# YPares/gaast

Measured on AMD Instinct MI355X. Metric: full-MV geometric products/sec (dim n); achieved HBM GB/s vs roofline, higher is better.
Workload: dtype f32; 1 GPU; R^12 full MV x MV geometric product, f32 (BASELINE configs[2]); dim=12, batch_per_gpu=65536, global_batch=65536

## Files before the change

gaast_amd/csrc/device/kernels_dense.hip.hpp:

```cpp
#pragma once
#include "kernels_common.hip.hpp"
#include "mfma32p_b_planes.hip.hpp"


namespace gaast {

template <typename T>
struct DenseArgs {
    const T* left;
    const T* right;
    T* out;
    int64_t left_stride, right_stride, out_stride;
    const uint32_t* left_map;
    const uint32_t* right_map;
    int left_count, right_count;
    int left_full, right_full;
    int left_contig, right_contig;
    const int32_t* out_map;
    int canon_left, canon_right;
    int n;
    uint32_t neg_hi, zero_hi;
    uint32_t neg_lo;
    int beta;
    const T* left_scale;
// ... 402 lines not shown
            auto one_step = [&](auto odd_tag, int a_hi) {
                constexpr bool ODD = decltype(odd_tag)::value;
                uint32_t sp = uint32_t(a_hi) >> 1;
                sp ^= sp >> 1;
                sp ^= sp >> 2;
                sp ^= sp >> 4;
                sp ^= sp >> 8;
                const uint32_t M = sp ^ (uint32_t(a_hi) & p.neg_hi);
                const uint32_t u = (__builtin_popcount(uint32_t(a_hi) & sp) ^
                                    __builtin_popcount(uint32_t(a_hi) & p.neg_hi)) & 1u;
                const uint32_t sbit = (u ^ uint32_t(__builtin_popcount(uint32_t(c_hi) & M))) & 1u;
                T sgn = sbit ? T(-1) : T(1);
                if (DEGENERATE) {
                    if (uint32_t(a_hi) & ~uint32_t(c_hi) & p.zero_hi) sgn = zero;
                }
                acc.template step<ODD, NEGLO>(As, Bs, a_hi, a_hi ^ c_hi, sgn);
            };
            const int half = LPI >> 1;
            for (int i = 0; i < half; ++i) one_step(std::false_type{}, (i << 1) | (__builtin_popcount(uint32_t(i)) & 1));
            for (int i = 0; i < half; ++i) one_step(std::true_type{}, (i << 1) | ((__builtin_popcount(uint32_t(i)) & 1) ^ 1));

            T* orow = p.out + (item0 + it) * p.out_stride;
#pragma unroll
            for (int i = 0; i < 16; ++i) store_result<T>(orow, om[i], acc.get(i), p.beta, out_scale, (c_hi << 4) + i);
        }
        __syncthreads();
    }
}


__device__ __forceinline__ constexpr int lo5_reorder_parity(int a, int b) {
    int par = 0;
    for (int p = 1; p < 5; ++p)
        if ((a >> p) & 1)
            for (int q = 0; q < p; ++q) par ^= (b >> q) & 1;
    return par;
}

__device__ __forceinline__ int mfma_b_pos(int m) {
    const int x = m >> 5, k = m & 31;
    const int lq = ((k & 1) << 2) | (k >> 3);
    return (x << 5) | (((lq ^ (x >> 1)) & 7) << 2) | ((k >> 1) & 3);
}

template <bool DEGENERATE, int THREADS, bool SCALED = false, bool CHAINED = false>
__global__ __launch_bounds__(THREADS) void k_gp_mfma32(DenseArgs<float> p) {
    const float* const left_scale = SCALED ? p.left_scale : nullptr;
    const float* const right_scale = SCALED ? p.right_scale : nullptr;
    const float* const out_scale = SCALED ? p.out_scale : nullptr;
    extern __shared__ __attribute__((aligned(16))) unsigned char smem_raw[];
    float* smem = reinterpret_cast<float*>(smem_raw);
    const int n = p.n;
    const int N = 1 << n;
    const int hbits = n - 5;
    const int H = 1 << hbits;
    const int WPI = H >> 5;
    const int IPB = (THREADS >> 6) / WPI;
    const int item_stride = 2 * N;
    const int tid = threadIdx.x;
    const int64_t item0 = int64_t(blockIdx.x) * IPB;
    const int nitems = int(p.batch - item0 < IPB ? p.batch - item0 : IPB);

    if (!p.left_full || !p.right_full) {
        for (int i = tid; i < nitems * item_stride; i += THREADS) smem[i] = 0.f;
        __syncthreads();
    }
    {
        if constexpr (CHAINED)
            stage_from_list<float, THREADS>(p, item0, nitems, smem, item_stride, smem + p.pre_scratch, tid);
        else
            stage_operands<float, THREADS>(p.left + item0 * p.left_stride, p.left_stride, p.left_map, p.left_count, p.left_contig,
                                       p.canon_left, smem, item_stride, nitems, tid, left_scale);
        stage_operands<float, THREADS>(p.right + item0 * p.right_stride, p.right_stride, p.right_map, p.right_count,
                                       p.right_contig, p.canon_right, smem + N, item_stride, nitems, tid, right_scale);
    }
    __syncthreads();

    const int wave = tid >> 6, lane = tid & 63;
    const int it = wave / WPI, tile = wave - it * WPI;
    if (it < nitems) {
        const float* As = smem + it * item_stride;
        const float* Bs = As + N;
        const int i = lane & 31, h = lane >> 5;
        const int c_hi = (tile << 5) | i;

        uint32_t amask[16];
        uint32_t aoff[16];
#pragma unroll
        for (int s2 = 0; s2 < 16; ++s2) {
            const int k = 2 * s2 + h;
            const int a_lo = i ^ k;
            int par = __builtin_popcount(uint32_t(a_lo & k) & p.neg_lo) & 1;
            for (int pp = 1; pp < 5; ++pp)
                if ((a_lo >> pp) & 1) par ^= __builtin_popcount(k & ((1 << pp) - 1)) & 1;
            amask[s2] = uint32_t(par) << 31;
            aoff[s2] = uint32_t(a_lo) << 2;
        }

        float16v acc;
#pragma unroll
        for (int r = 0; r < 16; ++r) acc[r] = 0.f;

        const unsigned char* As_b = reinterpret_cast<const unsigned char*>(As);
        const unsigned char* Bs_b = reinterpret_cast<const unsigned char*>(Bs);
        uint32_t bq[4];
#pragma unroll
        for (int q = 0; q < 4; ++q) bq[q] = (uint32_t(c_hi) << 7) | (uint32_t((((h << 2) | q) ^ (c_hi >> 1)) & 7) << 4);
        const uint32_t c_hi_u = uint32_t(c_hi) | 0x8000u;
        auto one_step = [&](int a_hi) {
            uint32_t sp = uint32_t(a_hi) >> 1;
            sp ^= sp >> 1;
            sp ^= sp >> 2;
            sp ^= sp >> 4;
            sp ^= sp >> 8;
            const uint32_t M = sp ^ (uint32_t(a_hi) & p.neg_hi);
            const uint32_t u = (__builtin_popcount(uint32_t(a_hi) & sp) ^
                                __builtin_popcount(uint32_t(a_hi) & p.neg_hi)) & 1u;
            const uint32_t bmask = uint32_t(__builtin_popcount(c_hi_u & (M | (u << 15)))) << 31;
            float bscale = 1.f;
            if (DEGENERATE) {
                if (uint32_t(a_hi) & ~uint32_t(c_hi) & p.zero_hi) bscale = 0.f;
            }
            float bv[16];
            const uint32_t sx = (uint32_t(a_hi) << 7) | (uint32_t((a_hi >> 1) & 7) << 4);
#pragma unroll
            for (int q = 0; q < 4; ++q) {
                const float4v v = *reinterpret_cast<const float4v*>(Bs_b + (bq[q] ^ sx));
                bv[4 * q + 0] = v.x; bv[4 * q + 1] = v.y; bv[4 * q + 2] = v.z; bv[4 * q + 3] = v.w;
            }
            const uint32_t abase = uint32_t(a_hi) << 7;
#pragma unroll
            for (int s2 = 0; s2 < 16; ++s2) {
                float a = *reinterpret_cast<const float*>(As_b + abase + aoff[s2]);
                a = __uint_as_float(__float_as_uint(a) ^ amask[s2]);
                float b = __uint_as_float(__float_as_uint(bv[s2]) ^ bmask);
                if (DEGENERATE) b *= bscale;
                acc = __builtin_amdgcn_mfma_f32_32x32x2f32(a, b, acc, 0, 0, 0);
            }
        };
        const int half = H >> 1;
        for (int t2 = 0; t2 < half; ++t2) one_step((t2 << 1) | (__builtin_popcount(uint32_t(t2)) & 1));
#pragma unroll
        for (int s2 = 0; s2 < 16; ++s2)
            amask[s2] ^= uint32_t((__builtin_popcount(uint32_t(s2)) + h) & 1) << 31;
        for (int t2 = 0; t2 < half; ++t2) one_step((t2 << 1) | ((__builtin_popcount(uint32_t(t2)) & 1) ^ 1));

        float* orow = p.out + (item0 + it) * p.out_stride;
        const int32_t* om = p.out_map + (c_hi << 5);
#pragma unroll
        for (int r = 0; r < 16; ++r) {
            const int c_lo = (r & 3) + 8 * (r >> 2) + 4 * h;
            store_result<float>(orow, om[c_lo], acc[r], p.beta, out_scale, (c_hi << 5) + c_lo);
        }
    }
}

template <int THREADS>
__device__ __forceinline__ void lds_barrier() {
    if (THREADS <= 64) {
        __builtin_amdgcn_wave_barrier();
        asm volatile("" ::: "memory");
    } else {
        asm volatile("s_waitcnt lgkmcnt(0)\n\ts_barrier" ::: "memory");
    }
}

typedef __attribute__((address_space(3))) unsigned char lds_u8;
typedef uint32_t uint4v __attribute__((ext_vector_type(4)));

__device__ __forceinline__ uint32_t xor3(uint32_t a, uint32_t b, uint32_t c) {
#if __has_builtin(__builtin_amdgcn_bitop3_b32)
    return __builtin_amdgcn_bitop3_b32(a, b, c, 0x96);
#else
    return a ^ b ^ c;
#endif
}

__device__ __forceinline__ constexpr int mfma16_k(int t) {
    constexpr int order[16] = {0, 3, 5, 6, 9, 10, 12, 15, 1, 2, 4, 7, 8, 11, 13, 14};
    return order[t];
}
static_assert(mfma16_k(1) == int(b_planes::s2_of_word(1)) && mfma16_k(7) == int(b_planes::s2_of_word(7)) && mfma16_k(8) == int(b_planes::s2_of_word(8)) &&
              mfma16_k(14) == int(b_planes::s2_of_word(14)), "the quad-plane B image stores the words in mfma16_k order");

template <bool DEGENERATE, int NDIM, bool SCALED = false, bool CHAINED = false>
__global__ __launch_bounds__(NDIM == 13 ? 512 : 256, NDIM <= 11 ? 2 : 1) void k_gp_mfma32p(DenseArgs<float> p) {
    const float* const left_scale = SCALED ? p.left_scale : nullptr;
    const float* const right_scale = SCALED ? p.right_scale : nullptr;
    const float* const out_scale = SCALED ? p.out_scale : nullptr;
    extern __shared__ __attribute__((aligned(16))) unsigned char smem_raw[];
    float* smem = reinterpret_cast<float*>(smem_raw);
    lds_u8* lds = (lds_u8*)smem_raw;
    constexpr int n = NDIM;
    constexpr int THREADS = NDIM == 13 ? 512 : 256;
    constexpr int N = 1 << n;
    constexpr int H = 1 << (n - 5);
    constexpr int WPI = H >> 5;
    constexpr int IPB = (THREADS >> 6) / WPI;
    constexpr int item_stride = 4 * N;
    constexpr uint32_t NEG = uint32_t(N) << 2;
    constexpr int PR = N / 4;
    constexpr int MPR = PR / THREADS;
    constexpr int ROWS = 2 * IPB;
    static_assert(MPR * ROWS == 8, "eight 16-byte pieces per thread and group");
    const int tid = threadIdx.x;
    const int64_t num_groups = (p.batch + IPB - 1) / IPB;
    const bool fast = !SCALED && !CHAINED && p.left_contig && p.right_contig && p.left_full && p.right_full;

    if (tid < 16) smem[IPB * item_stride + tid] = 0.f;

    uint32_t mw[2][MPR * 4];
    float4 pf[8];
    auto fetch = [&](int64_t g) {
        const int64_t it0 = g * IPB;
        const int cnt = int(p.batch - it0 < IPB ? p.batch - it0 : IPB);
#pragma unroll
        for (int r = 0; r < ROWS; ++r) {
            const int k = r % IPB;
            if (k < cnt) {
                const float* row = r < IPB ? p.left + (it0 + k) * p.left_stride : p.right + (it0 + k) * p.right_stride;
#pragma unroll
                for (int m = 0; m < MPR; ++m) pf[r * MPR + m] = reinterpret_cast<const float4*>(row)[tid + m * THREADS];
            }
        }
    };
    if (fast) {
#pragma unroll
        for (int m = 0; m < MPR; ++m) {
            const uint4 ml = reinterpret_cast<const uint4*>(p.left_map)[tid + m * THREADS];
            const uint4 mr = reinterpret_cast<const uint4*>(p.right_map)[tid + m * THREADS];
            mw[0][4 * m + 0] = ml.x; mw[0][4 * m + 1] = ml.y; mw[0][4 * m + 2] = ml.z; mw[0][4 * m + 3] = ml.w;
            mw[1][4 * m + 0] = mr.x; mw[1][4 * m + 1] = mr.y; mw[1][4 * m + 2] = mr.z; mw[1][4 * m + 3] = mr.w;
        }
        if (int64_t(blockIdx.x) < num_groups) fetch(blockIdx.x);
    }

    const int wave = tid >> 6, lane = tid & 63;
    const int it = wave / WPI, tile = wave - it * WPI;
    const int i = lane & 31, h = lane >> 5;
    const int c_hi = (tile << 5) | i;
    const uint32_t item_base = uint32_t(it) * uint32_t(item_stride) * 4u;

    constexpr bool ABS_A = NDIM <= 11 || (NDIM == 12 && !DEGENERATE);
    const uint32_t lds0 = ABS_A ? uint32_t(size_t(lds)) : 0u;
    uint32_t ak0[16];
#pragma unroll
    for (int t = 0; t < 16; ++t) {
        const int k = 2 * mfma16_k(t) + h;
        const int a_lo = i ^ k;
        int par = __builtin_popcount(uint32_t(a_lo & k) & p.neg_lo) & 1;
        for (int pp = 1; pp < 5; ++pp)
            if ((a_lo >> pp) & 1) par ^= __builtin_popcount(k & ((1 << pp) - 1)) & 1;
        ak0[t] = lds0 + item_base + (uint32_t(a_lo) << 2) + (par ? NEG : 0u);
    }
    const uint32_t b_base = item_base + 2u * NEG;
    constexpr uint32_t zero_block = uint32_t(IPB) * uint32_t(item_stride) * 4u;
    uint32_t bq[4];
#pragma unroll
    for (int q = 0; q < 4; ++q) {
        bq[q] = (uint32_t(c_hi) << 7) | (uint32_t((((h << 2) | q) ^ (c_hi >> 1)) & 7) << 4);
        if ((__builtin_popcount(uint32_t(c_hi)) & 1) && (((q >> 1) ^ h) & 1)) bq[q] ^= NEG;
    }
    const uint32_t c_hi_u = uint32_t(c_hi) | 0x8000u;
    auto sign_terms = [&](int a_hi, uint32_t& M, uint32_t& u) {
        const uint32_t sp = b_planes::suffix_parities(uint32_t(a_hi));
        M = sp ^ (uint32_t(a_hi) & p.neg_hi);
        u = (__builtin_popcount(uint32_t(a_hi) & sp) ^ __builtin_popcount(uint32_t(a_hi) & p.neg_hi)) & 1u;
    };
    auto block_sign = [&](int a_hi) -> uint32_t {
        uint32_t M, u;
        sign_terms(a_hi, M, u);
        return uint32_t(__builtin_popcount(c_hi_u & (M | (u << 15)))) & 1u;
    };
    constexpr int SIGN_WORDS = H <= 64 ? H / 32 : 0;
    constexpr bool XOR_STEP = NDIM == 12 && !DEGENERATE;
    if (XOR_STEP && (lds0 & ((16u << n) - 1u))) __builtin_trap();
    uint32_t dlt[XOR_STEP ? 7 : 1] = {0};
    uint32_t ud[XOR_STEP ? H / 32 : 1] = {0};
    if constexpr (XOR_STEP) {
#pragma unroll
        for (int t = 0; t < 7; ++t) dlt[t] = b_planes::delta(t, uint32_t(c_hi), p.neg_hi);
        static_assert(!XOR_STEP || (NEG == b_planes::kNeg && IPB == 1), "one item per workgroup, the -B image 16 KiB above +B");
#pragma unroll
        for (int w = 0; w < H / 32; ++w) {
            uint32_t bits = 0;
#pragma unroll 1
            for (int b = 0; b < 32; ++b) {
                uint32_t M, u0, u1;
                sign_terms(32 * w + b, M, u0);
                sign_terms(32 * w + b + 1, M, u1);
                bits |= (u0 ^ u1) << b;
            }
            ud[w] = __builtin_amdgcn_readfirstlane(bits);
        }
    }
    uint32_t sgn[SIGN_WORDS > 0 ? SIGN_WORDS : 1] = {0};
#pragma unroll
    for (int w = 0; w < SIGN_WORDS; ++w) {
        uint32_t bits = 0;
#pragma unroll 1
        for (int b = 0; b < 32; ++b) bits |= block_sign(32 * w + b) << b;
        sgn[w] = bits;
    }

    for (int64_t g = blockIdx.x; g < num_groups; g += gridDim.x) {
        const int64_t item0 = g * IPB;
        const int nitems = int(p.batch - item0 < IPB ? p.batch - item0 : IPB);
        if (fast) {
            auto stage_row = [&](int r, bool canon) {
                const int k = r % IPB, side = r / IPB;
                if (k < nitems) {
#pragma unroll
                    for (int m = 0; m < MPR; ++m) {
                        const float4 v = pf[r * MPR + m];
                        const float x[4] = {v.x, v.y, v.z, v.w};
#pragma unroll
                        for (int c = 0; c < 4; ++c) {
                            const uint32_t w = mw[side][4 * m + c];
                            float y = x[c];
                            if (canon) y = 0.f + y;
                            const uint32_t yb = __float_as_uint(y) ^ (w & 0x80000000u);
                            const uint32_t at = uint32_t(k) * uint32_t(item_stride * 4) + (side ? 2u * NEG : 0u) + (((w >> 16) & 0x7fffu) << 2);
                            *(__attribute__((address_space(3))) uint32_t*)(lds + at) = yb;
                            *(__attribute__((address_space(3))) uint32_t*)(lds + at + NEG) = yb ^ 0x80000000u;
                        }
                    }
                }
            };
#pragma unroll
            for (int r = 0; r < ROWS; ++r) {
                if constexpr (XOR_STEP) {
                    if (r / IPB ? p.canon_right : p.canon_left) stage_row(r, true);
                    else stage_row(r, false);
                } else {
                    stage_row(r, r / IPB ? p.canon_right : p.canon_left);
                }
            }
        } else {
            if (!p.left_full || !p.right_full) {
                for (int e = tid; e < nitems * item_stride; e += THREADS) smem[e] = 0.f;
                lds_barrier<THREADS>();
            }
            if constexpr (CHAINED)
                stage_from_list<float, THREADS>(p, item0, nitems, smem, item_stride, smem + p.pre_scratch, tid);
            else
                stage_operands<float, THREADS>(p.left + item0 * p.left_stride, p.left_stride, p.left_map, p.left_count, p.left_contig,
                                           p.canon_left, smem, item_stride, nitems, tid, left_scale);
            stage_operands<float, THREADS>(p.right + item0 * p.right_stride, p.right_stride, p.right_map, p.right_count,
                                           p.right_contig, p.canon_right, smem + 2 * N, item_stride, nitems, tid, right_scale);
            lds_barrier<THREADS>();
            constexpr int quads_per_item = N >> 1;
            for (int e = tid; e < nitems * quads_per_item; e += THREADS) {
                const int sit = e / quads_per_item, j = e - sit * quads_per_item;
                const int src = sit * item_stride + (j << 2) + ((j << 2) < N ? 0 : N);
                const float4v v = *reinterpret_cast<const float4v*>(smem + src);
                *reinterpret_cast<float4v*>(smem + src + N) = -v;
            }
        }
        lds_barrier<THREADS>();
        if (fast && g + gridDim.x < num_groups) fetch(g + gridDim.x);

        if (it < nitems) {
            float16v acc;
#pragma unroll
            for (int r = 0; r < 16; ++r) acc[r] = 0.f;
            uint32_t akc[XOR_STEP ? 1 : 16];
            uint32_t (&ak)[16] = *reinterpret_cast<uint32_t (*)[16]>(XOR_STEP ? ak0 : akc);
            if constexpr (!XOR_STEP) {
#pragma unroll
                for (int t = 0; t < 16; ++t) ak[t] = ak0[t];
            }

            auto step = [&](int a_hi, int j, uint32_t sxs) {
                uint32_t bw[16], aw[16];
#pragma unroll
                for (int q = 0; q < 4; ++q) {
                    uint32_t addr = b_base + (bq[q] ^ sxs);
                    if (DEGENERATE) addr = (uint32_t(a_hi) & ~uint32_t(c_hi) & p.zero_hi) ? zero_block : addr;
                    const uint4v v = *(__attribute__((address_space(3))) const uint4v*)(lds + addr);
                    bw[4 * q + 0] = v.x; bw[4 * q + 1] = v.y; bw[4 * q + 2] = v.z; bw[4 * q + 3] = v.w;
                }
#pragma unroll
                for (int t = 0; t < 16; ++t)
                    aw[t] = ABS_A ? *(__attribute__((address_space(3))) const uint32_t*)size_t(ak[t] + uint32_t(j << 7))
                                  : *(__attribute__((address_space(3))) const uint32_t*)(lds + ak[t] + uint32_t(j << 7));
#pragma unroll
                for (int t = 0; t < 16; ++t)
                    acc = __builtin_amdgcn_mfma_f32_32x32x2f32(__uint_as_float(aw[t]), __uint_as_float(bw[t]), acc, 0, 0, 0);
                asm volatile("" ::: "memory");
            };
            if constexpr (SIGN_WORDS > 0 && NDIM <= 11) {
                uint32_t awin[4];
                uint4v qb[2];
                auto b_quad = [&](int a_hi, int q, uint32_t sxs) -> uint4v {
                    uint32_t addr = b_base + (bq[q] ^ sxs);
                    if (DEGENERATE) addr = (uint32_t(a_hi) & ~uint32_t(c_hi) & p.zero_hi) ? zero_block : addr;
                    return *(__attribute__((address_space(3))) const uint4v*)(lds + addr);
                };
                auto a_word = [&](int t, int j) -> uint32_t {
                    return ABS_A ? *(__attribute__((address_space(3))) const uint32_t*)size_t(ak[t] + uint32_t(j << 7))
                                 : *(__attribute__((address_space(3))) const uint32_t*)(lds + ak[t] + uint32_t(j << 7));
                };
                auto sx_of = [&](int a_hi) -> uint32_t {
                    uint32_t sx = __builtin_amdgcn_readfirstlane((uint32_t(a_hi) << 7) | (uint32_t((a_hi >> 1) & 7) << 4));
                    asm("" : "+s"(sx));
                    return sx;
                };
                uint32_t sxs = ((sgn[0] & 1u) << (n + 2)) | sx_of(0);
                qb[0] = b_quad(0, 0, sxs);
#pragma unroll
                for (int t = 0; t < 3; ++t) awin[t] = a_word(t, 0);
#pragma unroll
                for (int w = 0; w < SIGN_WORDS; ++w) {
                    uint32_t sw = sgn[w];
                    const uint32_t next_word_bit0 = w + 1 < SIGN_WORDS ? (sgn[w + 1 < SIGN_WORDS ? w + 1 : w] & 1u) : 0u;
#pragma unroll 1
                    for (int c = 0; c < 2; ++c) {
                        const int a0 = 32 * w + 16 * c;
#pragma unroll
                        for (int j = 0; j < 16; ++j) {
                            const int a_hi = a0 + j;
                            const uint32_t nbit = j < 15 ? (sw >> (j + 1)) & 1u : (c == 0 ? (sw >> 16) & 1u : next_word_bit0);
                            const uint32_t nsxs = (nbit << (n + 2)) | sx_of(a_hi + 1);
#pragma unroll
                            for (int t = 0; t < 16; ++t) {
                                const int m = 16 * j + t;
                                const int t3 = (t + 3) & 15, j3 = j + ((t + 3) >> 4);
                                awin[(m + 3) & 3] = a_word(t3, j3);
                                if ((t & 3) == 0) {
                                    const int q = t >> 2;
                                    qb[(q + 1) & 1] = q < 3 ? b_quad(a_hi, q + 1, sxs) : b_quad(a_hi + 1, 0, nsxs);
                                }
                                __builtin_amdgcn_sched_barrier(0);
                                const uint4v bqv = qb[(t >> 2) & 1];
                                const uint32_t bwv = (t & 3) == 0 ? bqv.x : (t & 3) == 1 ? bqv.y : (t & 3) == 2 ? bqv.z : bqv.w;
                                acc = __builtin_amdgcn_mfma_f32_32x32x2f32(__uint_as_float(awin[m & 3]), __uint_as_float(bwv), acc, 0, 0, 0);
                                __builtin_amdgcn_sched_barrier(0);
                            }
                            sxs = nsxs;
                        }
                        sw >>= 16;
#pragma unroll
                        for (int t = 0; t < 16; ++t) ak[t] += 16u << 7;
                    }
                }
            } else if constexpr (XOR_STEP) {
                uint32_t xe = lds0 + (b_base | b_planes::xe0(uint32_t(c_hi), uint32_t(h)));
                uint32_t xo = lds0 + (b_base | b_planes::xo0(uint32_t(c_hi), uint32_t(h)));
#pragma unroll 1
                for (int c = 0; c < H / 64; ++c) {
                    const uint32_t udw[2] = {c == 0 ? ud[0] : ud[2], c == 0 ? ud[1] : ud[3]};
#pragma unroll
                    for (int j = 0; j < 64; ++j) {
                        uint32_t bw[16], aw[16];
#pragma unroll
                        for (int q = 0; q < 4; ++q) {
                            const uint4v v = *(__attribute__((address_space(3))) const uint4v*)size_t((q & 2 ? xo : xe) + uint32_t(q & 1) * b_planes::kQuadStride);
                            bw[4 * q + 0] = v.x; bw[4 * q + 1] = v.y; bw[4 * q + 2] = v.z; bw[4 * q + 3] = v.w;
                        }
#pragma unroll
                        for (int t = 0; t < 16; ++t)
                            aw[t] = *(__attribute__((address_space(3))) const uint32_t*)size_t(ak[t] + uint32_t(j << 7));
#pragma unroll
                        for (int t = 0; t < 16; ++t)
                            acc = __builtin_amdgcn_mfma_f32_32x32x2f32(__uint_as_float(aw[t]), __uint_as_float(bw[t]), acc, 0, 0, 0);
                        asm volatile("" ::: "memory");
                        uint32_t su = __builtin_amdgcn_readfirstlane(((udw[j >> 5] >> (j & 31)) & 1u) << (n + 2));
                        asm("" : "+s"(su));
                        const uint32_t d = dlt[j < 63 ? __builtin_ctz(~uint32_t(j)) : 6];
                        xe = xor3(xe, d, su);
                        xo = xor3(xo, d, su);
                    }
#pragma unroll
                    for (int t = 0; t < 16; ++t) ak[t] ^= 64u << 7;
                }
            } else {
                for (int a0 = 0; a0 < H; a0 += 8) {
#pragma unroll
                    for (int j = 0; j < 8; ++j) {
                        const int a_hi = a0 + j;
                        const uint32_t sx = (uint32_t(a_hi) << 7) | (uint32_t((a_hi >> 1) & 7) << 4);
                        step(a_hi, j, (block_sign(a_hi) << (n + 2)) | sx);
                    }
#pragma unroll
                    for (int t = 0; t < 16; ++t) ak[t] += 8u << 7;
                }
            }

            float* orow = p.out + (item0 + it) * p.out_stride;
            if constexpr (XOR_STEP) {
                const int32_t* om = p.out_map + (c_hi << 5);
                int32_t ow[16];
#pragma unroll
                for (int r = 0; r < 16; ++r) ow[r] = om[(r & 3) + 8 * (r >> 2) + 4 * h];
                asm volatile("" ::: "memory");
                auto put = [&](bool signs, bool beta) {
#pragma unroll
                    for (int r = 0; r < 16; ++r) {
                        const int32_t w = ow[r];
                        if (w < 0) continue;
                        float v = acc[r];
                        if (out_scale) v = v * out_scale[(c_hi << 5) + (r & 3) + 8 * (r >> 2) + 4 * h];
                        if (signs && (w & 0x40000000)) v = beta ? -v : 0.f + (-v);
                        float* dst = orow + (signs ? w & 0x3fffffff : w);
                        *dst = beta ? *dst + v : v;
                    }
                };
                if (p.out_signs) put(true, p.beta != 0);
                else put(false, p.beta != 0);
            } else {
                const int32_t* om = p.out_map + (c_hi << 5);
#pragma unroll
                for (int r = 0; r < 16; ++r) {
                    const int c_lo = (r & 3) + 8 * (r >> 2) + 4 * h;
                    store_result<float>(orow, om[c_lo], acc[r], p.beta, out_scale, (c_hi << 5) + c_lo);
                }
            }
        }
        lds_barrier<THREADS>();
    }
}

typedef double double4m __attribute__((ext_vector_type(4)));

template <typename T>
struct Mfma16x4;
template <>
struct Mfma16x4<double> {
    typedef double4m acc_t;
    static constexpr int SHIFT = 3;
    static __device__ __forceinline__ acc_t mma(double a, double b, acc_t c) { return __builtin_amdgcn_mfma_f64_16x16x4f64(a, b, c, 0, 0, 0); }
    static __device__ __forceinline__ int row(int kq, int r) { return 4 * r + kq; }
    static constexpr bool QUAD = false;
    static __device__ __forceinline__ constexpr int k_of(int kq, int s) { return 4 * s + kq; }
    static __device__ __forceinline__ double flip(double v, uint32_t bit31) { return __hiloint2double(__double2hiint(v) ^ int(bit31), __double2loint(v)); }
};
template <>
struct Mfma16x4<float> {
    typedef float4v acc_t;
    static constexpr int SHIFT = 2;
    static __device__ __forceinline__ acc_t mma(float a, float b, acc_t c) { return __builtin_amdgcn_mfma_f32_16x16x4f32(a, b, c, 0, 0, 0); }
    static __device__ __forceinline__ int row(int kq, int r) { return 4 * kq + r; }
    static constexpr bool QUAD = true;
    static __device__ __forceinline__ constexpr int k_of(int kq, int s) {
        constexpr int tab[4][4] = {{0, 3, 5, 6}, {9, 10, 12, 15}, {1, 2, 4, 7}, {8, 11, 13, 14}};
        return tab[kq][s];
    }
    static __device__ __forceinline__ float flip(float v, uint32_t bit31) { return __uint_as_float(__float_as_uint(v) ^ bit31); }
};

template <typename T, bool DEGENERATE, int NDIM, int MODE, bool SCALED = false, bool CHAINED = false>
__global__ __launch_bounds__(64 << (NDIM - 8)) __attribute__((amdgpu_waves_per_eu(2))) void k_gp_mfma16x4(DenseArgs<T> p) {
    constexpr bool FAST = MODE >= 1;
    static_assert(!(SCALED && MODE != 0), "a rescaled basis runs on the general staging and stores");
    const T* const left_scale = SCALED ? p.left_scale : nullptr;
    const T* const right_scale = SCALED ? p.right_scale : nullptr;
    const T* const out_scale = SCALED ? p.out_scale : nullptr;
    extern __shared__ __attribute__((aligned(16))) unsigned char smem_raw[];
    T* smem = reinterpret_cast<T*>(smem_raw);
    lds_u8* lds = (lds_u8*)smem_raw;
    typedef __attribute__((address_space(3))) T lds_t;
    typedef Mfma16x4<T> MM;
    constexpr int ES = MM::SHIFT;
    constexpr int n = NDIM;
    constexpr int N = 1 << n;
    constexpr int H = 1 << (n - 4);
    constexpr int THREADS = 64 << (n - 8);
#ifndef GAAST_MFMA16X4_PAD_MAXN
#define GAAST_MFMA16X4_PAD_MAXN 9
#endif
    constexpr int PAD_A = NDIM <= GAAST_MFMA16X4_PAD_MAXN ? 16 : 0;
    constexpr int A_EL = PAD_A ? 2 * N : 0, B_EL = PAD_A ? 0 : 2 * N;
    constexpr int item_stride = 4 * N + 32;
    constexpr uint32_t NEG = uint32_t(N) << ES;
    constexpr uint32_t A_BASE = uint32_t(A_EL) << ES, NEG_A = uint32_t(N + PAD_A) << ES;
    constexpr uint32_t B_BASE = uint32_t(B_EL) << ES;
    constexpr int BS = 4 + ES;
    const int tid = threadIdx.x;
    if (tid < 16) smem[4 * N + PAD_A + tid] = T(0);

    const int tile = tid >> 6, lane = tid & 63;
    const int i = lane & 15, kq = lane >> 4;
    const int c_hi = (tile << 4) | i;

    uint32_t ak[4], bk[4];
#pragma unroll
    for (int s = 0; s < 4; ++s) {
        const int k = MM::k_of(kq, s);
        const int a_lo = i ^ k;
        int par = __builtin_popcount(uint32_t(a_lo & k) & p.neg_lo) & 1;
        for (int pp = 1; pp < 4; ++pp)
            if ((a_lo >> pp) & 1) par ^= __builtin_popcount(k & ((1 << pp) - 1)) & 1;
        ak[s] = A_BASE + (uint32_t(a_lo) << ES) + (par ? NEG_A : 0u);
        if (MM::QUAD) {
            bk[s] = (uint32_t(c_hi) << BS) | (uint32_t(kq ^ (((c_hi >> 2) & 1) << 1)) << 4);
            if ((__builtin_popcount(uint32_t(c_hi)) & 1) && kq >= 2) bk[s] ^= NEG;
        } else {
            bk[s] = (uint32_t(c_hi) << BS) | ((uint32_t((c_hi >> 1) & 7) << (1 + ES)) ^ (uint32_t(k) << ES));
            if ((__builtin_popcount(uint32_t(c_hi)) & __builtin_popcount(uint32_t(k))) & 1) bk[s] ^= NEG;
        }
    }
    constexpr int SW = (H + 31) / 32, SB = H < 32 ? H : 32;
    uint32_t sign_bits[SW], zero_bits[SW];
#pragma unroll
    for (int w = 0; w < SW; ++w) {
        uint32_t sb = 0, zb = 0;
#pragma unroll 1
        for (int b = 0; b < SB; ++b) {
            const int a_hi = 32 * w + b;
            uint32_t sp = uint32_t(a_hi) >> 1;
            sp ^= sp >> 1;
            sp ^= sp >> 2;
            sp ^= sp >> 4;
            const uint32_t M = sp ^ (uint32_t(a_hi) & p.neg_hi);
            const uint32_t u = (__builtin_popcount(uint32_t(a_hi) & sp) ^ __builtin_popcount(uint32_t(a_hi) & p.neg_hi)) & 1u;
            sb |= ((u ^ uint32_t(__builtin_popcount(uint32_t(c_hi) & M))) & 1u) << b;
            if (DEGENERATE) zb |= ((uint32_t(a_hi) & ~uint32_t(c_hi) & p.zero_hi) ? 1u : 0u) << b;
        }
        sign_bits[w] = sb;
        zero_bits[w] = zb;
    }
    constexpr uint32_t zero_block = uint32_t(4 * N + PAD_A) << ES;
#pragma unroll
    for (int s = 0; s < 4; ++s) bk[s] |= B_BASE;
    uint32_t ooff[4], osg[4];
    bool ook[4];
    T osc[4];
#pragma unroll
    for (int r = 0; r < 4; ++r) {
        const int32_t w = p.out_map[(c_hi << 4) + MM::row(kq, r)];
        ook[r] = w >= 0;
        ooff[r] = uint32_t(w & 0x3fffffff) << ES;
        osg[r] = (uint32_t(w) & 0x40000000u) << 1;
        osc[r] = (SCALED && out_scale) ? out_scale[(c_hi << 4) + MM::row(kq, r)] : T(1);
    }

    constexpr int CPP = 16 >> ES;
    constexpr int PPT = 4 / CPP;
    static_assert((N / CPP) == PPT * THREADS, "four components of each row per thread");
    uint32_t wa[4] = {0, 0, 0, 0}, wb[4] = {0, 0, 0, 0}, sa[4] = {0, 0, 0, 0}, sb[4] = {0, 0, 0, 0};
    T pf_l[4], pf_r[4];
    const bool same_src = CHAINED && p.pre_left == p.right && p.pre_left_stride == p.right_stride && p.pre_left_len == N &&
                          p.pre_right_len <= THREADS;
    T pf_x = T(0);
    auto fetch = [&](int64_t item) {
#pragma unroll
        for (int m = 0; m < PPT; ++m) {
            uint32_t o = uint32_t(tid + m * THREADS) * 16u;
            asm volatile("" : "+v"(o));
            if constexpr (!CHAINED) {
                const uint4 xl = *reinterpret_cast<const uint4*>(reinterpret_cast<const unsigned char*>(p.left + item * p.left_stride) + o);
                __builtin_memcpy(&pf_l[m * CPP], &xl, 16);
            }
            const uint4 xr = *reinterpret_cast<const uint4*>(reinterpret_cast<const unsigned char*>(p.right + item * p.right_stride) + o);
            __builtin_memcpy(&pf_r[m * CPP], &xr, 16);
        }
        if constexpr (CHAINED) {
            if (same_src && tid < p.pre_right_len) pf_x = p.pre_right[item * p.pre_right_stride + tid];
        }
    };
    if (FAST) {
#pragma unroll
        for (int e = 0; e < 4; ++e) {
            const int idx = ((e / CPP) * THREADS + tid) * CPP + (e % CPP);
            const uint32_t mr = p.right_map[idx];
            if constexpr (!CHAINED) {
                const uint32_t ml = p.left_map[idx];
                wa[e] = A_BASE + (((ml >> 16) & 0x7fffu) << ES);
                sa[e] = ml & 0x80000000u;
            }
            wb[e] = B_BASE + (((mr >> 16) & 0x7fffu) << ES);
            sb[e] = mr & 0x80000000u;
        }
        if (int64_t(blockIdx.x) < p.batch) fetch(blockIdx.x);
    }

    constexpr bool LIST_CACHE = CHAINED && FAST && (NDIM == 8 || NDIM == 9);
    constexpr bool LC_PACKED = NDIM != 8;
    constexpr int LW = NDIM + 1;
    bool list_cached = LIST_CACHE && same_src && p.pre_width == 12 && p.pre_rows == 4 * THREADS && p.pre_row_scale == nullptr;
    uint32_t ce[(LIST_CACHE && LC_PACKED) ? 4 : 1][(LIST_CACHE && LC_PACKED) ? LW : 1];
    const lds_t *cl[(LIST_CACHE && !LC_PACKED) ? 4 : 1][(LIST_CACHE && !LC_PACKED) ? LW : 1], *cr[(LIST_CACHE && !LC_PACKED) ? 4 : 1][(LIST_CACHE && !LC_PACKED) ? LW : 1];
    uint32_t crow[4] = {0, 0, 0, 0};
    if constexpr (LIST_CACHE) {
        if (list_cached) {
            const uint32_t ll = uint32_t(p.pre_left_len), rl = uint32_t(p.pre_right_len);
            bool pads_only = true;
#pragma unroll
            for (int rr = 0; rr < 4; ++rr) {
                crow[rr] = p.pre_row_map[tid + rr * THREADS];
#pragma unroll
                for (int t = 0; t < 12; ++t) {
                    const uint32_t e = p.pre_entries[t * (4 * THREADS) + tid + rr * THREADS];
                    if (t < LW) {
                        const uint32_t la = (uint32_t(p.pre_scratch) + (e & 0x7fffu)) << ES;
                        const uint32_t ra = (uint32_t(p.pre_scratch) + ll + ((e >> 16) & 0x7fffu) + ((e >> 31) ? rl + 1u : 0u)) << ES;
                        if constexpr (LC_PACKED) {
                            ce[rr][t < LW ? t : 0] = la | (ra << 16);
                        } else {
                            cl[rr][t < LW ? t : 0] = (const lds_t*)(lds + la);
                            cr[rr][t < LW ? t : 0] = (const lds_t*)(lds + ra);
                        }
                    } else {
                        pads_only = pads_only && (e & 0x7fffu) == ll + rl;
                    }
                }
            }
            list_cached = __all(pads_only) != 0;
        }
    }
    auto cached_list = [&]() {
        if constexpr (LIST_CACHE) {
#pragma unroll
            for (int rr = 0; rr < 4; ++rr) {
                T lv[LW], rv[LW];
#pragma unroll
                for (int t = 0; t < LW; ++t) {
                    if constexpr (LC_PACKED) {
                        uint32_t e = ce[rr][t];
                        asm volatile("" : "+v"(e));
                        lv[t] = *(const lds_t*)(lds + (e & 0xffffu));
                        rv[t] = *(const lds_t*)(lds + (e >> 16));
                    } else {
                        lv[t] = *cl[rr][t];
                        rv[t] = *cr[rr][t];
                    }
                }
                T acc = T(0);
#pragma unroll
                for (int t = 0; t < LW; ++t) acc = acc + lv[t] * rv[t];
                uint32_t w = crow[rr];
                asm volatile("" : "+v"(w));
                const uint32_t pos = (w >> 16) & 0x7fffu;
                const T val = list_flip<T>(acc, w & 0x80000000u);
                smem[A_EL + pos] = val;
                smem[A_EL + pos + N + PAD_A] = -val;
            }
        }
    };
    for (int64_t item = blockIdx.x; item < p.batch; item += gridDim.x) {
        if (FAST) {
#pragma unroll
            for (int e = 0; e < 4; ++e) {
                T yr = pf_r[e];
                if constexpr (CHAINED) {
                    if (same_src) {
                        const int idx = ((e / CPP) * THREADS + tid) * CPP + (e % CPP);
                        smem[p.pre_scratch + idx] = p.pre_canon_left ? T(0) + yr : yr;
                    }
                } else {
                    T yl = pf_l[e];
                    if (p.left_signs) yl = MM::flip(yl, sa[e]);
                    *(lds_t*)(lds + wa[e]) = yl;
                    *(lds_t*)(lds + wa[e] + NEG_A) = -yl;
                }
                yr = MM::flip(yr, sb[e]);
                *(lds_t*)(lds + wb[e]) = yr;
                *(lds_t*)(lds + wb[e] + NEG) = -yr;
            }
            if constexpr (CHAINED) {
                if (same_src) {
                    if (tid < p.pre_right_len) {
                        const T x = p.pre_canon_right ? T(0) + pf_x : pf_x;
                        smem[p.pre_scratch + N + tid] = x;
                        smem[p.pre_scratch + N + p.pre_right_len + 1 + tid] = -x;
                    }
                    if (tid == 0) smem[p.pre_scratch + N + p.pre_right_len] = T(0);
                } else {
                    list_fill_scratch<T, THREADS>(p, item, 1, smem + p.pre_scratch, tid);
                }
                if (!p.left_full) {
                    for (int e = tid; e < N; e += THREADS) {
                        smem[A_EL + e] = T(0);
                        smem[A_EL + N + PAD_A + e] = T(0);
                    }
                }
                if (THREADS > 64) __syncthreads();
                else asm volatile("s_waitcnt vmcnt(0) lgkmcnt(0)" ::: "memory");
            } else {
                lds_barrier<THREADS>();
            }
            fetch(item + gridDim.x < p.batch ? item + gridDim.x : item);
            if constexpr (CHAINED) {
                if (list_cached) cached_list();
                else list_eval_rows<T, THREADS>(p, 1, smem + A_EL, item_stride, smem + p.pre_scratch, tid, N + PAD_A);
                lds_barrier<THREADS>();
            }
        } else {
            if (!p.left_full || !p.right_full) {
                for (int e = tid; e < 4 * N + PAD_A; e += THREADS) smem[e] = T(0);
                lds_barrier<THREADS>();
            }
            if constexpr (CHAINED)
                stage_from_list<T, THREADS>(p, item, 1, smem + A_EL, item_stride, smem + p.pre_scratch, tid);
            else
                stage_operands<T, THREADS>(p.left + item * p.left_stride, p.left_stride, p.left_map, p.left_count, p.left_contig,
                                           p.canon_left, smem + A_EL, item_stride, 1, tid, left_scale);
            stage_operands<T, THREADS>(p.right + item * p.right_stride, p.right_stride, p.right_map, p.right_count,
                                       p.right_contig, p.canon_right, smem + B_EL, item_stride, 1, tid, right_scale);
            lds_barrier<THREADS>();
            for (int e = tid; e < 2 * N; e += THREADS) {
                if (e < N) smem[B_EL + N + e] = -smem[B_EL + e];
                else smem[A_EL + PAD_A + e] = -smem[A_EL + e - N];
            }
            lds_barrier<THREADS>();
        }

        typename MM::acc_t acc = {T(0), T(0), T(0), T(0)};
        auto load_ops = [&](uint32_t sxs, uint32_t zero, const uint32_t (&abase)[4], int joff, T (&av)[4], T (&bv)[4]) {
            if constexpr (MM::QUAD) {
                uint32_t addr = bk[0] ^ sxs;
                if (DEGENERATE) addr = zero ? zero_block : addr;
                const float4v q = *(__attribute__((address_space(3))) const float4v*)(lds + addr);
                bv[0] = q[0]; bv[1] = q[1]; bv[2] = q[2]; bv[3] = q[3];
#pragma unroll
                for (int s = 0; s < 4; ++s) av[s] = *(const lds_t*)(lds + abase[s] + uint32_t(joff << BS));
            } else {
#pragma unroll
                for (int s = 0; s < 4; ++s) {
                    uint32_t addr = bk[s] ^ sxs;
                    if (DEGENERATE) addr = zero ? zero_block : addr;
                    bv[s] = *(const lds_t*)(lds + addr);
// ... 399 lines not shown
```

Baseline: 4.384 million products/s.

## Defer output stores into next group's MFMA loop to overlap writes

For the unscaled XOR-step path with beta==0 and no output signs, the accumulator results are held in registers instead of being stored right away. They are written out during steps 8-23 of the next group's first MFMA chunk, interleaved one store per step, and the final group is flushed after the loop. Output offsets are precomputed once per thread as byte offsets, and an SGPR base is used for the global store. The aim is to hide global store latency behind matrix work, at the cost of extra registers for the pending values.

Result: no change. 4.407 million products/s, median of 6 (+0.5%).

```diff
diff --git a/gaast_amd/csrc/device/kernels_dense.hip.hpp b/gaast_amd/csrc/device/kernels_dense.hip.hpp
--- a/gaast_amd/csrc/device/kernels_dense.hip.hpp
+++ b/gaast_amd/csrc/device/kernels_dense.hip.hpp
@@ -728,8 +728,29 @@
         for (int b = 0; b < 32; ++b) bits |= block_sign(32 * w + b) << b;
         sgn[w] = bits;
     }
-
-    for (int64_t g = blockIdx.x; g < num_groups; g += gridDim.x) {
+    constexpr bool DEFER = XOR_STEP && !SCALED;
+    constexpr int STORE_STEP0 = 8;
+    int32_t owb[DEFER ? 16 : 1] = {0};
+    float pend[DEFER ? 16 : 1] = {0.f};
+    const bool defer = DEFER && p.beta == 0 && !p.out_signs;
+    if constexpr (DEFER) {
+        const int32_t* om = p.out_map + (c_hi << 5);
+#pragma unroll
+        for (int r = 0; r < 16; ++r) {
+            const int32_t w = om[(r & 3) + 8 * (r >> 2) + 4 * h];
+            owb[r] = w < 0 ? -1 : w << 2;
+        }
+    }
+    auto store_pending = [&](int r, int64_t item) {
+        uint64_t prow = reinterpret_cast<uint64_t>(p.out + item * p.out_stride);
+        asm volatile("" : "+s"(prow));
+        int32_t zero;
+        asm volatile("s_mov_b32 %0, 0" : "=s"(zero));
+        if (owb[r] >= zero) *reinterpret_cast<__attribute__((address_space(1))) float*>(prow + uint32_t(owb[r] + zero)) = pend[r];
+    };
+
+    int64_t g = blockIdx.x;
+    for (; g < num_groups; g += gridDim.x) {
         const int64_t item0 = g * IPB;
         const int nitems = int(p.batch - item0 < IPB ? p.batch - item0 : IPB);
         if (fast) {
@@ -876,6 +897,7 @@
 #pragma unroll 1
                 for (int c = 0; c < H / 64; ++c) {
                     const uint32_t udw[2] = {c == 0 ? ud[0] : ud[2], c == 0 ? ud[1] : ud[3]};
+                    const bool store_now = defer && g != int64_t(blockIdx.x) && c == 0;
 #pragma unroll
                     for (int j = 0; j < 64; ++j) {
                         uint32_t bw[16], aw[16];
@@ -891,6 +913,12 @@
                         for (int t = 0; t < 16; ++t)
                             acc = __builtin_amdgcn_mfma_f32_32x32x2f32(__uint_as_float(aw[t]), __uint_as_float(bw[t]), acc, 0, 0, 0);
                         asm volatile("" ::: "memory");
+                        if constexpr (DEFER) {
+                            if (j >= STORE_STEP0 && j < STORE_STEP0 + 16) {
+                                if (store_now) store_pending(j - STORE_STEP0, g - gridDim.x);
+                                asm volatile("" ::: "memory");
+                            }
+                        }
                         uint32_t su = __builtin_amdgcn_readfirstlane(((udw[j >> 5] >> (j & 31)) & 1u) << (n + 2));
                         asm("" : "+s"(su));
                         const uint32_t d = dlt[j < 63 ? __builtin_ctz(~uint32_t(j)) : 6];
@@ -915,12 +943,12 @@
 
             float* orow = p.out + (item0 + it) * p.out_stride;
             if constexpr (XOR_STEP) {
-                const int32_t* om = p.out_map + (c_hi << 5);
-                int32_t ow[16];
-#pragma unroll
-                for (int r = 0; r < 16; ++r) ow[r] = om[(r & 3) + 8 * (r >> 2) + 4 * h];
-                asm volatile("" ::: "memory");
                 auto put = [&](bool signs, bool beta) {
+                    const int32_t* om = p.out_map + (c_hi << 5);
+                    int32_t ow[16];
+#pragma unroll
+                    for (int r = 0; r < 16; ++r) ow[r] = om[(r & 3) + 8 * (r >> 2) + 4 * h];
+                    asm volatile("" ::: "memory");
 #pragma unroll
                     for (int r = 0; r < 16; ++r) {
                         const int32_t w = ow[r];
@@ -932,7 +960,12 @@
                         *dst = beta ? *dst + v : v;
                     }
                 };
-                if (p.out_signs) put(true, p.beta != 0);
+                if (defer) {
+                    if constexpr (DEFER) {
+#pragma unroll
+                        for (int r = 0; r < 16; ++r) pend[r] = acc[r];
+                    }
+                } else if (p.out_signs) put(true, p.beta != 0);
                 else put(false, p.beta != 0);
             } else {
                 const int32_t* om = p.out_map + (c_hi << 5);
@@ -944,6 +977,12 @@
             }
         }
         lds_barrier<THREADS>();
+    }
+    if constexpr (DEFER) {
+        if (defer && int64_t(blockIdx.x) < num_groups) {
+#pragma unroll
+            for (int r = 0; r < 16; ++r) store_pending(r, g - gridDim.x);
+        }
     }
 }
 
```
